# daisy9542/yolo-puncture

Measured on AMD Instinct MI355X. Metric: images/sec, higher is better.
Workload: dtype bf16

## Files before the change

### include/yolop.h

```cpp
#ifndef YOLOP_H
#define YOLOP_H

#include <stddef.h>
#include <stdint.h>

#ifdef __cplusplus
extern "C" {
#endif

#define YP_OK 0
#define YP_ERR_ARG -1
#define YP_ERR_STATE -2
#define YP_ERR_HIP -3
#define YP_ERR_WEIGHT -4

#define YP_BF16 0
#define YP_F32 1

#define YP_TASK_DETECT 0
#define YP_TASK_SEGMENT 1

#define YP_NM 32
#define YP_MAX_MASKS 480
#define YP_ID_MASKS_FRAMES_BUDGET (1ull << 30)
// ... 143 lines not shown
int yp_debug_op_cfg(const yp_engine* e, int i, int* cfg);
int yp_debug_last_store_form(void);
int yp_debug_max_workgroups(int n);
int yp_debug_conv_families(int* base, int* num_cfgs, int cap);
int yp_debug_ablation(int v);
int yp_debug_head_clocks(uint64_t* out8);
int yp_debug_attention(const void* qkv_dev, void* o_dev, int dtype, int B, int N, int nh, int kd, int hd, int q_stride, int q_coff, int o_stride,
                       int o_coff, int wgs, int* kernel_out, void* stream);
int yp_debug_attention_form(const void* qkv_dev, void* o_dev, int dtype, int B, int N, int nh, int kd, int hd, int q_stride, int q_coff, int o_stride,
                            int o_coff, int wgs, int form, int* kernel_out, void* stream);
int yp_debug_attention_f32(const void* qkv_dev, void* o_dev, int B, int N, int nh, int kd, int hd, int q_stride, int q_coff, int o_stride, int o_coff,
                           int wgs, int f32_stream, int* kernel_out, void* stream);
int yp_debug_conv_s2(const void* x_dev, const void* w_dev, const float* bias_dev, const void* res_dev, void* y_dev, int out_f32, int B, int H,
                     int W, int Cin, int Cout, int silu, int cfg, int lds_weights, int64_t* lds_out, char* kernel_out, int kernel_cap,
                     void* stream);
int yp_debug_topk_anchors(const uint32_t* const mk_dev[3], int B, const int hw[3][2], int k, int32_t* sel_out_dev, uint32_t* thr_out_dev, void* stream);
int yp_debug_head_branch_clocks(uint64_t* out8);
int yp_debug_head_winners(yp_engine* e, int32_t* sel_host, float* box_host, float* coeff_host);
int yp_debug_contour_clocks(uint64_t* out12);
int yp_debug_pwsp_clocks(uint64_t* out32);

int yp_tuning_source(const yp_engine* e);

int yp_debug_host_selftest(yp_engine* e);
int yp_debug_graph_info(const yp_engine* e, int64_t* out6);
int yp_debug_head_positions(yp_engine* e, int64_t* out6);
int yp_debug_marker(void* stream);

int yp_set_graph(yp_engine* e, int enable);

// ... 5 lines not shown
```

### yolo-puncture_amd/csrc/common.h

```cpp
#pragma once
#include <hip/hip_runtime.h>
#include <stdint.h>
#include <atomic>
#include <cstdlib>
#include <initializer_list>
#include <string>
#include <type_traits>
#include <vector>

namespace yp {

enum DType { DT_BF16 = 0, DT_F32 = 1 };
enum Act { ACT_NONE = 0, ACT_SILU = 1, ACT_RELU = 2 };

enum OpKind {
    OP_STEM = 0,
    OP_CONV = 1,
    OP_DWCONV = 2,
    OP_POOL5 = 3,
    OP_UPSAMPLE = 4,
    OP_ATTN = 5,
    OP_HEAD = 6,
    OP_CONVT = 7,
    OP_AMAX = 9,
// ... 297 lines not shown
template <class F> auto with_res_f32(const ConvParams& p, F f) {
    if (p.out_f32) return f(std::false_type{}, std::true_type{});
    if (p.res) return f(std::true_type{}, std::false_type{});
    return f(std::false_type{}, std::false_type{});
}
inline std::string res_f32_args(const ConvParams& p) { return with_res_f32(p, [](auto res, auto f32) { return bool_args({res, f32}); }); }
inline bool conv_store_side_ok(const ConvParams& p) {
    if ((p.Cout & 3) || (p.y_stride & 3) || (p.y_coff & 3) || (p.res && ((p.res_stride & 3) || (p.res_coff & 3)))) return false;
    if (p.res && p.out_f32) return false;
    return p.x_bytes < (1ull << 31) && p.w_bytes < (1ull << 31) && p.y_bytes < (1ull << 31);
}
extern const ConvFamily conv_dma_family, conv_halo_family, conv_halo_p_family, conv_dma_p_family, conv_dma_lc_family, conv_halo_s2_family,
    conv_tile1_family, conv_wreg_family, conv_pxd_family, conv_ks_family, conv_wres_family, conv_wrs_family;
constexpr int kNumConvFamilies = 12;
extern const ConvFamily* const kConvFamilies[kNumConvFamilies];
int conv_halo_s2_pw_cfg(const ConvParams& p);
size_t conv_halo_s2_lds_bytes(const ConvParams& p, int c);
int conv_halo_s2_lds_weights(int on);
hipError_t launch_dwconv(const DwParams& p, int dtype, hipStream_t st);
std::string dwconv_kernel_name(const DwParams& p, int dtype);
hipError_t launch_stem(const StemParams& p, int dtype, hipStream_t st);
std::string stem_kernel_name(const StemParams& p, int dtype);
hipError_t launch_pool5(const PoolParams& p, int dtype, hipStream_t st);
hipError_t launch_sppf_pool3(const PoolParams& p, int dtype, hipStream_t st);
bool sppf_pool3_fits(const PoolParams& p, int dtype);
bool dwconv_mfma_valid(const DwParams& p, int dtype);
hipError_t launch_dwconv_mfma(const DwParams& p, hipStream_t st);
const char* dwconv_mfma_kernel_name(const DwParams& p);
hipError_t launch_upsample(const UpParams& p, int dtype, hipStream_t st);
enum AttnForm { ATTN_FORM_AUTO = 0, ATTN_FORM_STREAM = 1, ATTN_FORM_STREAM_WIDE = 3 };
inline bool attn_form_valid(int form) { return form == ATTN_FORM_AUTO || form == ATTN_FORM_STREAM || form == ATTN_FORM_STREAM_WIDE; }
// ... 144 lines not shown
```

### yolo-puncture_amd/csrc/conv_halo_s2.hip

```cpp
#include "common.h"

namespace yp {

constexpr int kS2WregMaxVgprs = 144;

template <int FM, int FN, int WGM, int WGN, int NSH, bool HAS_RES, bool OUT_F32, bool PW2, int NCH>
__device__ __forceinline__ void conv_halo_s2_body(const ConvParams& p, const int tiles_h, const int tiles_w, const int ntiles, const int G) {
    constexpr int NW = WGM * WGN;
    constexpr int TH = WGM * FM, BN = WGN * FN * 16;
    constexpr int HR = 2 * TH + 1;
    constexpr int HP = HR * 33;
    constexpr int H_INSTR = (HP * 4 + 63) / 64;
    constexpr int LH = (H_INSTR + NW - 1) / NW;
    constexpr int HB = H_INSTR * 1024;
    constexpr int S = FM * FN;
    constexpr bool WREG = NCH > 0;
    static_assert(!WREG || (!PW2 && 9 * NCH * FN * 4 <= kS2WregMaxVgprs), "register-weights form");
    static_assert(NSH == 3, "wait selection below is written for a 3-slot ring");
    static_assert((NSH - 2) * LH + 2 * S < 64, "vmcnt immediate");

    extern __shared__ __attribute__((aligned(1024))) unsigned char smem[];
    unsigned char* const Hs = smem;
    unsigned char* const dump = smem + NSH * HB;
    unsigned char* const Wres = dump + 1024;

    const int tid = threadIdx.x, lane = tid & 63;
    const int wave = __builtin_amdgcn_readfirstlane(tid >> 6);
    const int wm = wave % WGM, wn = wave / WGM;
    const int fr = lane & 15, fc = lane >> 4;
    const int nchunk = WREG ? NCH : p.Cin >> 5;

    const int bid = xcd_remap(blockIdx.x, gridDim.x);
// ... 48 lines not shown
                for (int a = 0; a < FN; ++a) {
                    const int rw = t * BN + wn * (FN * 16) + a * 16 + fr;
                    wr[c][t][a] = *(const bf16x8*)(Hs + swz64((unsigned)(rw * 64 + fc * 16)));
                }
            __builtin_amdgcn_s_waitcnt(0xc07f);
            __builtin_amdgcn_s_barrier();
        }
#pragma unroll
        for (int c = 0; c < NCH; ++c)
#pragma unroll
            for (int t = 0; t < 9; ++t)
#pragma unroll
                for (int a = 0; a < FN; ++a) asm volatile("" : "+v"(wr[c][t][a]));
    }

    unsigned char* const W2s = Wres + (size_t)9 * nchunk * BN * 64;
    float bias2[FN][4];
    if (PW2) {
        static_assert(!PW2 || BN == 64, "the fused trailing 1x1 is written for a 64-wide intermediate and output");
        const __amdgpu_buffer_rsrc_t w2rs = __builtin_amdgcn_make_buffer_rsrc((void*)p.w2, 0, (int)p.w2_bytes, 0x00020000);
        for (int ii = wave; ii < BN * 8 / 64; ii += NW) {
            const int s = ii * 64 + lane;
            const int row = s >> 3, pc = s & 7;
            const int c8 = pc ^ ((row >> 1) & 7);
            const unsigned voff = (unsigned)((row * p.Kpad2 + c8 * 8) * 2);
            __builtin_amdgcn_raw_ptr_buffer_load_lds(w2rs, (lds_void*)(W2s + ii * 1024), 16, voff, 0, 0, 0);
        }
#pragma unroll
        for (int a = 0; a < FN; ++a) {
            const int co = wn * (FN * 16) + a * 16 + fc * 4;
#pragma unroll
            for (int r = 0; r < 4; ++r) bias2[a][r] = (co + r < p.C2) ? p.bias2[co + r] : 0.f;
        }
    }

    unsigned hconst[LH];
    auto set_tile = [&](int tile) {
        int t = tile;
        const int tw = t % tiles_w; t /= tiles_w;
// ... 108 lines not shown

        if (PW2) {
            unsigned char* tb = Hs + ((rd_slot == 0) ? NSH - 1 : rd_slot - 1) * HB;
            __builtin_amdgcn_s_barrier();
#pragma unroll
            for (int r = 0; r < FM; ++r) {
                const int px = (wm * FM + r) * 16 + fr;
#pragma unroll
                for (int a = 0; a < FN; ++a) {
                    const int co = wn * (FN * 16) + a * 16 + fc * 4;
                    __attribute__((aligned(8))) __bf16 o[4];
                    float sv[4] = {acc[a][r][0], acc[a][r][1], acc[a][r][2], acc[a][r][3]};
                    if (p.act == ACT_SILU) silu4_packed(sv);
#pragma unroll
                    for (int i = 0; i < 4; ++i) o[i] = (__bf16)sv[i];
                    asm volatile("ds_write_b64 %0, %1" ::"v"((unsigned)(size_t)(__attribute__((address_space(3))) unsigned char*)(tb + px * 128 + (((co >> 3) ^ ((px >> 1) & 7)) * 16) + (co & 7) * 2)),
                                 "v"(*(const unsigned long long*)o) : "memory");
                }
            }
            asm volatile("s_waitcnt lgkmcnt(0)" ::: "memory");
            __builtin_amdgcn_s_barrier();
#pragma unroll
            for (int a = 0; a < FN; ++a)
#pragma unroll
                for (int r = 0; r < FM; ++r) acc[a][r] = f32x4{bias2[a][0], bias2[a][1], bias2[a][2], bias2[a][3]};
#pragma unroll
            for (int ss = 0; ss < 2; ++ss) {
                bf16x8 w2f[FN], t2f[FM];
#pragma unroll
                for (int a = 0; a < FN; ++a) {
                    const int rw = wn * (FN * 16) + a * 16 + fr;
                    w2f[a] = *(const bf16x8*)(W2s + rw * 128 + (((ss * 4 + fc) ^ ((rw >> 1) & 7)) * 16));
                }
#pragma unroll
                for (int r = 0; r < FM; ++r) {
                    const int px = (wm * FM + r) * 16 + fr;
                    t2f[r] = *(const bf16x8*)(tb + px * 128 + (((ss * 4 + fc) ^ ((px >> 1) & 7)) * 16));
                }
#pragma unroll
                for (int a = 0; a < FN; ++a)
#pragma unroll
                    for (int r = 0; r < FM; ++r) acc[a][r] = __builtin_amdgcn_mfma_f32_16x16x32_bf16(w2f[a], t2f[r], acc[a][r], 0, 0, 0);
            }
        }
        {
            int t = tile;
            const int tw = t % tiles_w; t /= tiles_w;
            const int th = t % tiles_h;
            const int b = t / tiles_h;
            const int wo = tw * 16 + fr;
            uint2 rres[FM][FN];
            if (HAS_RES) {
// ... 41 lines not shown
    wait_vmcnt<0>();
}

template <int FM, int FN, int WGM, int WGN, int NSH, bool HAS_RES, bool OUT_F32, bool PW2>
__global__ __launch_bounds__(WGM * WGN * 64) void conv_halo_s2_kernel(const ConvParams p, const int tiles_h, const int tiles_w,
                                                                    const int ntiles, const int G) {
    conv_halo_s2_body<FM, FN, WGM, WGN, NSH, HAS_RES, OUT_F32, PW2, 0>(p, tiles_h, tiles_w, ntiles, G);
}
template <int FM, int FN, int WGM, int WGN, int NSH, bool HAS_RES, bool OUT_F32, bool PW2, int NCH>
__global__ __launch_bounds__(WGM * WGN * 64) void conv_halo_s2_kernel(const ConvParams p, const int tiles_h, const int tiles_w,
                                                                    const int ntiles, const int G) {
    static_assert(NCH > 0, "the ninth argument is a register-weights form's chunk count");
    conv_halo_s2_body<FM, FN, WGM, WGN, NSH, HAS_RES, OUT_F32, PW2, NCH>(p, tiles_h, tiles_w, ntiles, G);
}

enum { S2_PW2 = 1, S2_WREG = 2 };
template <int FM, int FN, int WGM, int WGN, int FORM = 0> struct S2 : Cfg<FM, FN, WGM, WGN, 3> {
    static constexpr int TH = WGM * FM, BN = WGN * FN * 16;
    static constexpr bool pw2 = FORM & S2_PW2, wreg = FORM & S2_WREG;
    static constexpr size_t lds(int Cin, bool with_pw2 = false) {
        const size_t ring = (size_t)3 * (((2 * TH + 1) * 33 * 4 + 63) / 64) * 1024 + 1024;
        if (wreg) return std::max(ring, (size_t)9 * BN * 64);
        return ring + (size_t)9 * (Cin / 32) * BN * 64 + (with_pw2 ? (size_t)BN * 128 : 0);
    }
};
using S2Forms = CfgList<
    S2<2, 2, 4, 2, S2_PW2>,
    S2<1, 2, 4, 2, S2_PW2>,
    S2<2, 2, 4, 1>,
    S2<1, 2, 4, 1>,
    S2<2, 4, 4, 2>,
    S2<1, 2, 4, 2, S2_WREG>,
    S2<2, 2, 4, 2, S2_WREG>,
    S2<2, 2, 2, 4, S2_WREG>>;
constexpr int kNumS2 = 5;

static std::atomic<int>& s2_lds_weights_ref() {
    static std::atomic<int> v{env_on("YOLOP_S2_LDS_WEIGHTS") ? 1 : 0};
    return v;
}
int conv_halo_s2_lds_weights(int on) { return on < 0 ? s2_lds_weights_ref().load() : s2_lds_weights_ref().exchange(on ? 1 : 0); }

static int halo_s2_form(const ConvParams& p, int c) {
    if (c < 0 || c >= kNumS2) return -1;
    if (c > 1 || p.C2 > 0 || s2_lds_weights_ref().load()) return c;
    if ((p.Cin % 32) != 0 || 9 * (p.Cin / 32) * 2 * 4 > kS2WregMaxVgprs) return c;
    if (c == 0) return 6;
    return p.Cout > 96 ? 7 : 5;
}
static std::string conv_halo_s2_symbol(const ConvParams& p, int c) {
    return with_cfg<S2Forms>(halo_s2_form(p, c), [&](auto k) {
        if (k.wreg) return cfg_symbol("conv_halo_s2_kernel", k, res_f32_args(p) + bool_args({false}) + "," + std::to_string(p.Cin / 32));
        return cfg_symbol("conv_halo_s2_kernel", k, p.C2 > 0 ? bool_args({false, false, true}) : res_f32_args(p) + bool_args({false}));
    });
}

static bool conv_halo_s2_cfg_valid(const ConvParams& p, int c) {
    if (p.ks != 3 || p.stride != 2 || p.pad != 1 || p.up != 1 || (p.Cin % 32) != 0 || (p.Kpad != 9 * p.Cin)) return false;
    if ((p.H & 1) || (p.W & 1) || p.Ho * 2 != p.H || p.Wo * 2 != p.W) return false;
    if (!conv_store_side_ok(p)) return false;
    return with_cfg<S2Forms>(halo_s2_form(p, c), [&](auto k) {
        using K = decltype(k);
        const int cpad = (p.Cout + 31) / 32 * 32;
        if (K::BN > cpad) return false;
        if (K::lds(p.Cin) > 160 * 1024) return false;
        const long covered = (long)((p.Ho + K::TH - 1) / K::TH * K::TH) * ((p.Wo + 15) / 16 * 16);
// ... 1 lines not shown
    });
}

template <bool HAS_RES, bool OUT_F32, bool PW2, int... WCH, int FM, int FN, int WGM, int WGN, int FORM>
static hipError_t launch_halo_s2_var(S2<FM, FN, WGM, WGN, FORM> k, const ConvParams& p, hipStream_t st) {
    static_assert(sizeof...(WCH) == 0 || (FN == 2 && 9 * 2 * FN * 4 <= kS2WregMaxVgprs && 9 * 3 * FN * 4 > kS2WregMaxVgprs), "the chunk counts instantiated are those halo_s2_form admits");
    constexpr int TH = k.TH, BN = k.BN;
    const size_t sh = k.lds(p.Cin, PW2);
    const int B = p.M / (p.Ho * p.Wo);
    const int tiles_h = (p.Ho + TH - 1) / TH, tiles_w = (p.Wo + 15) / 16, ntiles = (p.Cout + BN - 1) / BN;
    const int num_tiles = B * tiles_h * tiles_w;
    const int per_cu = sizeof...(WCH) > 0 ? 1 : (int)std::max<size_t>(1, std::min<size_t>(2, (160 * 1024) / sh));
    int G = (256 * per_cu) / ntiles;
    if (G < 1) G = 1;
    if (G > num_tiles) G = num_tiles;
    auto kern = conv_halo_s2_kernel<FM, FN, WGM, WGN, 3, HAS_RES, OUT_F32, PW2, WCH...>;
    static size_t granted = 0;
    if (hipError_t e = allow_dynamic_lds((const void*)kern, sh, granted)) return e;
    hipLaunchKernelGGL(kern, dim3(G * ntiles), dim3(WGM * WGN * 64), sh, st, p, tiles_h, tiles_w, ntiles, G);
    return hipGetLastError();
}

int conv_halo_s2_pw_cfg(const ConvParams& p) {
    if (p.w2 == nullptr && p.C2 == 0) return -1;
    if (p.Cout != 64 || p.C2 != 64 || p.Kpad2 != 64 || p.res || p.out_f32) return -1;
    for (int c : {0, 1}) {
        ConvParams q = p;
        q.Cout = p.C2;
        if (!conv_halo_s2_cfg_valid(q, c)) continue;
        if (with_cfg<S2Forms>(c, [&](auto k) { return k.lds(p.Cin, true); }) > 160 * 1024) continue;
        return c;
    }
    return -1;
}

size_t conv_halo_s2_lds_bytes(const ConvParams& p, int c) {
    return with_cfg<S2Forms>(halo_s2_form(p, c), [&](auto k) { return k.lds(p.Cin); });
}

static hipError_t launch_conv_halo_s2(const ConvParams& p, int c, hipStream_t st) {
    return with_cfg<S2Forms>(halo_s2_form(p, c), [&](auto k) {
        using K = decltype(k);
        if constexpr (K::wreg) {
            return with_res_f32(p, [&](auto res, auto f32) {
                if (p.Cin == 32) return launch_halo_s2_var<res, f32, false, 1>(k, p, st);
                if (p.Cin == 64) return launch_halo_s2_var<res, f32, false, 2>(k, p, st);
                return hipErrorInvalidValue;
            });
        } else {
            if (p.C2 > 0) {
                if constexpr (K::pw2) return launch_halo_s2_var<false, false, true>(k, p, st);
                else return hipErrorInvalidValue;
            }
            return with_res_f32(p, [&](auto res, auto f32) { return launch_halo_s2_var<res, f32, false>(k, p, st); });
        }
    });
}

// ... 6 lines not shown
```

### yolo-puncture_amd/csrc/engine.hip

```cpp
#include "../../include/yolop.h"
#include "common.h"
#include <algorithm>
#include <array>
#include <chrono>

#include <cmath>
#include <cstdarg>
#include <cstdio>
#include <cstring>
#include <cstdlib>
#include <dlfcn.h>
#include <fcntl.h>
#include <fstream>
#include <map>
#include <sstream>
#include <memory>

using namespace yp;

static thread_local char g_err[512] = "";
static int fail(int code, const char* fmt, ...) {
    va_list ap;
    va_start(ap, fmt);
    vsnprintf(g_err, sizeof(g_err), fmt, ap);
// ... 22 lines not shown
    size_t arena_bytes = 0;
    int proto_t = -1;
    void* mask_ws = nullptr;
    void* head_ws = nullptr;
    size_t head_ws_bytes = 0;
    size_t mask_ws_bytes = 0;
    bool use_graph = false;
    bool graph_auto = false;
    std::map<std::array<int, 3>, bool> auto_replay;
    bool fuse = true;
    int attn_form = ATTN_FORM_AUTO;
    int attn_f32_stream = ATTN_F32_GENERIC;
    bool tail = false;
    bool narrow_store = false;
    bool sparse_head = true;
    void* sp_ws = nullptr; size_t sp_ws_bytes = 0;
    bool tune = true;
    int tune_source = 0;
    hipStream_t own_stream = nullptr;
    hipEvent_t ev_in = nullptr;
    hipGraphExec_t gexec = nullptr;
    hipGraph_t gsrc = nullptr;
    bool use_lanes = true;
    int n_captures = 0;
    int g_nodes = 0, g_edges = 0, g_edges_expected = 0;
    hipStream_t last_stream = nullptr; bool have_last = false;
    struct LaneStep { int op = -1; std::vector<int> waits; bool fork = false; bool record = false; };
    std::vector<LaneStep> lane_steps;
    std::vector<int> lanes_used;
    int n_lanes = 1;
// ... 772 lines not shown

static int tail_absorbed(const yp_engine& e, const Op& o, int m[3]) {
    if (o.fuse_tail < 0) return 0;
    m[0] = e.ops[o.fuse_tail].fuse_dw; m[1] = o.fuse_tail; m[2] = o.tail_amax;
    return o.tail_amax >= 0 ? 3 : 2;
}
static std::string tail_admit(const yp_engine& e, const Op& o, int& cfg) {
    return e.tail && e.ops[o.fuse_tail].form == FORM_DWPW ? dwpw_admit(e, o, cfg) : "";
}
static void tail_views(const yp_engine& e, const Op& o, View& in, View& extra) {
    in = e.ops[e.ops[o.fuse_tail].fuse_dw].in;
    if (o.tail_amax >= 0) extra = e.ops[o.tail_amax].out;
}

static int s2pw_absorbed(const yp_engine&, const Op& o, int m[3]) { return link1(o.fuse_pre, m); }
static std::string s2pw_admit(const yp_engine& e, const Op& o, int& cfg) {
    const ConvParams q = conv_params(e, o);
    const int c = conv_halo_s2_pw_cfg(q);
    if (c < 0) return "";
    cfg = conv_halo_s2_family.base + c;
    return conv_halo_s2_family.symbol(q, c);
}
static void s2pw_views(const yp_engine& e, const Op& o, View& in, View&) { in = e.ops[o.fuse_pre].in; }
static hipError_t s2pw_launch(const yp_engine& e, const Op& o, const RunArgs&, hipStream_t st) {
    return conv_halo_s2_family.launch(conv_params(e, o), o.cfg - conv_halo_s2_family.base, st);
}

static int front_absorbed(const yp_engine&, const Op& o, int m[3]) {
    m[0] = o.stem_op; m[1] = o.fuse_pre;
    return o.stem_op >= 0 && o.fuse_pre >= 0 ? 2 : 0;
}
static std::string front_admit(const yp_engine& e, const Op& o, int&) {
    return e.weights[e.ops[o.stem_op].widx].d_w2 && frontend_valid(front_params(e, o, nullptr)) ? "frontend_kernel" : "";
// ... 959 lines not shown
    std::unique_ptr<yp_engine> e(new yp_engine());
    e->desc = *desc; e->device = device; e->dtype = desc->dtype;
    e->fuse = !env_on("YOLOP_NO_FUSE");
    e->tail = env_on("YOLOP_TAIL");
    if (const char* v = std::getenv("YOLOP_ATTN_FORM")) {
        if (!strcmp(v, "stream")) e->attn_form = ATTN_FORM_STREAM;
        else if (!strcmp(v, "stream_wide")) e->attn_form = ATTN_FORM_STREAM_WIDE;
        else if (*v && strcmp(v, "auto")) return fail(YP_ERR_ARG, "YOLOP_ATTN_FORM=%s (auto | stream | stream_wide)", v);
    }
    if (const char* v = std::getenv("YOLOP_ATTN_F32")) {
        if (!strcmp(v, "stream")) e->attn_f32_stream = ATTN_F32_STREAM;
        else if (!strcmp(v, "stream_wide")) e->attn_f32_stream = ATTN_F32_STREAM_WIDE;
        else if (*v) return fail(YP_ERR_ARG, "YOLOP_ATTN_F32=%s (stream | stream_wide, or unset)", v);
    }
    e->sparse_head = !env_on("YOLOP_DENSE_HEAD");
    e->narrow_store = env_on("YOLOP_NARROW_STORE");
    int rc = build_graph(*e);
    if (rc != YP_OK) return rc;
    for (const Op& o : e->ops)
        for (const View* v : {&o.in, &o.out, &o.res})
            if (v->t >= 0 && o.kind != OP_STEM && ((v->C & 7) || (v->coff & 7)) && !e->tensors[v->t].f32)
                return fail(YP_ERR_ARG, "op %s: channel slice (%d,%d) is not a multiple of 8", o.name.c_str(), v->coff, v->C);
    *out = e.release();
    return YP_OK;
}

int yp_destroy(yp_engine* e) {
    if (!e) return YP_OK;
    if (e->finalized || e->arena) { (void)hipSetDevice(e->device); (void)hipDeviceSynchronize(); }
    for (auto& w : e->weights) { if (w.d_w) (void)hipFree(w.d_w); if (w.d_w2) (void)hipFree(w.d_w2); if (w.d_b) (void)hipFree(w.d_b); }
// ... 600 lines not shown
    const int before = conv_halo_s2_lds_weights(lds_weights ? 1 : 0);
    const bool ok = f.valid(p, cfg - f.base);
    hipError_t err = hipSuccess;
    if (lds_out) *lds_out = (int64_t)conv_halo_s2_lds_bytes(p, cfg - f.base);
    if (ok && kernel_out && kernel_cap > 0) std::snprintf(kernel_out, (size_t)kernel_cap, "%s", f.symbol(p, cfg - f.base).c_str());
    if (ok && !host_only) {
        hipStream_t st = (hipStream_t)stream;
        err = f.launch(p, cfg - f.base, st);
        if (err == hipSuccess) err = hipStreamSynchronize(st);
    }
    conv_halo_s2_lds_weights(before);
    if (!ok)
        return fail(YP_ERR_ARG, "yp_debug_conv_s2: configuration %d does not admit B %d, H %d, W %d, Cin %d, Cout %d%s%s%s", cfg, B, H, W, Cin, Cout,
                    res_dev ? ", residual" : "", out_f32 ? ", fp32 output" : "", lds_weights ? ", weights in LDS" : "");
    if (err != hipSuccess) return fail(YP_ERR_HIP, "yp_debug_conv_s2: %s", hipGetErrorString(err));
    return YP_OK;
}

int yp_tuning_source(const yp_engine* e) {
    if (!e) return YP_ERR_ARG;
    return e->tune_source;
}

int yp_debug_graph_info(const yp_engine* e, int64_t* out6) {
    if (!e || !out6) return fail(YP_ERR_ARG, "yp_debug_graph_info: null argument");
    out6[0] = e->n_captures; out6[1] = e->g_nodes; out6[2] = e->g_edges; out6[3] = e->g_edges_expected;
    out6[4] = (int64_t)e->lanes_used.size() + 1; out6[5] = e->gexec ? 1 : 0;
    return YP_OK;
}

// ... 501 lines not shown
```

### yolo-puncture_amd/engine.py

```python
from __future__ import annotations

import ctypes as C
import os
from typing import Dict, List, Optional, Tuple

import numpy as np
import torch

from .weights import fold_state

_LIB: Optional[C.CDLL] = None
_HERE = os.path.dirname(os.path.abspath(__file__))
LIB_PATH = os.environ.get("YOLOP_LIB") or os.path.join(_HERE, "libyolop.so")

YP_BF16, YP_F32 = 0, 1
TASK_DETECT, TASK_SEGMENT = 0, 1
OP_KINDS = {0: "stem", 1: "conv", 2: "dwconv", 3: "pool5", 4: "upsample", 5: "attn", 6: "head", 7: "convT", 8: "pool3", 9: "amax"}
FORMS = ("plain", "dwpw", "dwpw_tail", "s2pw", "frontend", "c2f", "scdown", "pwsp", "cls_out")


class ModelDesc(C.Structure):
    _fields_ = [("variant", C.c_int), ("nc", C.c_int), ("task", C.c_int), ("dtype", C.c_int), ("max_det", C.c_int), ("family", C.c_int)]


# ... 31 lines not shown
    lib.yp_mask_contours_large_workspace.restype = C.c_size_t
    lib.yp_mask_contours_large.argtypes = [vp, C.c_int, C.c_int, C.c_int, C.c_int, C.c_int, vp, vp, vp, C.c_int, vp, C.c_int, C.c_int, C.c_int, vp,
                                           C.c_size_t, vp]
    lib.yp_mask_contours_large.restype = C.c_int
    lib.yp_plan.argtypes = [vp, C.c_int, C.c_int, C.c_int]
    lib.yp_max_batch.argtypes = [vp, C.c_int, C.c_int]
    lib.yp_max_batch.restype = C.c_int
    lib.yp_debug_topk_anchors.argtypes = [C.POINTER(vp), C.c_int, C.POINTER(C.c_int), C.c_int, vp, vp, vp]
    lib.yp_debug_topk_anchors.restype = C.c_int
    lib.yp_debug_attention.argtypes = [vp, vp] + [C.c_int] * 11 + [ip, vp]
    lib.yp_debug_attention.restype = C.c_int
    lib.yp_debug_attention_form.argtypes = [vp, vp] + [C.c_int] * 12 + [ip, vp]
    lib.yp_debug_attention_form.restype = C.c_int
    lib.yp_debug_conv_s2.argtypes = [vp, vp, vp, vp, vp] + [C.c_int] * 9 + [C.POINTER(C.c_int64), C.c_char_p, C.c_int, vp]
    lib.yp_debug_conv_s2.restype = C.c_int
    lib.yp_set_attention_form.argtypes = [vp, C.c_int]
    lib.yp_set_attention_form.restype = C.c_int
    lib.yp_debug_attention_f32.argtypes = [vp, vp] + [C.c_int] * 11 + [ip, vp]
    lib.yp_debug_attention_f32.restype = C.c_int
    lib.yp_set_attention_f32_stream.argtypes = [vp, C.c_int]
    lib.yp_set_attention_f32_stream.restype = C.c_int
    lib.yp_op_info.argtypes = [vp, C.c_int, C.c_char_p, C.c_int, ip, C.POINTER(C.c_double), C.POINTER(C.c_double)]
    lib.yp_op_output.argtypes = [vp, C.c_int, ip, ip, ip]
    lib.yp_op_kernel.argtypes = [vp, C.c_int, C.c_char_p, C.c_int]
    lib.yp_op_fusion.argtypes = [vp, C.c_int, ip, ip]
    lib.yp_op_fusion.restype = C.c_int
    lib.yp_debug_op_form.argtypes = [vp, C.c_int, ip, ip, C.c_int]
    lib.yp_debug_op_form.restype = C.c_int
    lib.yp_run_op.argtypes = [vp, C.c_int, vp, vp, vp, vp, vp]
    lib.yp_tensor_write.argtypes = [vp, C.c_int, C.c_int, C.c_int, vp]
# ... 50 lines not shown
    for fn in ("yp_comm_unique_id", "yp_comm_create", "yp_allgather", "yp_comm_destroy"):
        getattr(lib, fn).restype = C.c_int
    for fn in ("yp_create", "yp_destroy", "yp_weight_count", "yp_weight_info", "yp_set_weight", "yp_finalize",
               "yp_forward", "yp_proto", "yp_masks", "yp_plan", "yp_op_info", "yp_op_output", "yp_op_input", "yp_tensor_count",
               "yp_tensor_info", "yp_tensor_read", "yp_profile", "yp_set_graph", "yp_run_op", "yp_tensor_write",
               "yp_op_kernel", "yp_set_autotune", "yp_debug_force_conv_cfg", "yp_debug_ablation"):
        getattr(lib, fn).restype = C.c_int
    if path is None:
        _LIB = lib
    return lib


EXPORTS = ["yp_last_error", "yp_create", "yp_destroy", "yp_weight_count", "yp_weight_info", "yp_set_weight",
           "yp_finalize", "yp_forward", "yp_proto", "yp_masks", "yp_id_mask_resized", "yp_plan", "yp_op_info", "yp_op_output", "yp_op_input", "yp_op_fusion",
           "yp_tensor_count", "yp_tensor_info", "yp_tensor_read", "yp_profile", "yp_set_graph", "yp_run_op",
           "yp_tensor_write", "yp_op_kernel", "yp_set_autotune", "yp_tuning_export", "yp_tuning_import", "yp_set_nms", "yp_set_nms_options", "yp_debug_force_conv_cfg", "yp_debug_op_cfg", "yp_debug_op_form", "yp_debug_last_store_form", "yp_debug_max_workgroups", "yp_debug_conv_families", "yp_debug_ablation", "yp_debug_head_clocks", "yp_debug_head_branch_clocks", "yp_debug_head_winners", "yp_debug_contour_clocks", "yp_debug_pwsp_clocks", "yp_debug_host_selftest", "yp_debug_graph_info", "yp_tuning_source", "yp_debug_head_positions", "yp_debug_marker", "yp_max_batch", "yp_debug_topk_anchors", "yp_debug_attention", "yp_debug_attention_form", "yp_debug_attention_f32", "yp_debug_conv_s2", "yp_set_attention_form", "yp_set_attention_f32_stream", "yp_letterbox", "yp_letterbox_batch", "yp_masks_frames", "yp_masks_frames_input", "yp_id_masks_frames", "yp_id_masks_frames_workspace", "yp_mask_contours",
           "yp_mask_contours_scaled", "yp_mask_contours_large_workspace", "yp_mask_contours_large", "yp_comm_unique_id", "yp_comm_create", "yp_allgather", "yp_comm_destroy",
           "yp_u2net_create", "yp_u2net_destroy", "yp_u2net_weight_count", "yp_u2net_weight_info", "yp_u2net_set_weight", "yp_u2net_finalize",
           "yp_u2net_forward", "yp_u2net_forward_crops", "yp_u2net_set_graph", "yp_u2net_tensor_count", "yp_u2net_tensor_info", "yp_u2net_tensor_read",
           "yp_u2net_op_count", "yp_u2net_op_info",
           "yp_cls_create", "yp_cls_destroy", "yp_cls_weight_count", "yp_cls_weight_info", "yp_cls_set_weight", "yp_cls_finalize",
           "yp_cls_forward", "yp_cls_set_graph", "yp_cls_tensor_count", "yp_cls_tensor_info", "yp_cls_tensor_read"]


MAX_ANCHORS = 294912
MAX_MASKS = 480
ID_MASKS_FRAMES_BUDGET = 1 << 30
ATTENTION_FORMS = {"auto": 0, "stream": 1, "stream_wide": 3}


ATTENTION_F32 = {"generic": 0, "stream": 1}
# ... 88 lines not shown
                              C.c_void_p(res.data_ptr()) if res is not None else None, C.c_void_p(y.data_ptr()), int(bool(out_f32)), B, H, W, Cin, Cout,
                              int(bool(silu)), int(cfg), int(bool(lds_weights)), None, None, 0, C.c_void_p(_stream_ptr(x.device)))
    if rc < 0:
        raise YolopError(lib.yp_last_error().decode())
    return y


def conv_s2_admits(cfg: int, B: int, H: int, W: int, Cin: int, Cout: int, res: bool = False, out_f32: bool = False,
                   lds_weights: bool = False) -> Tuple[bool, int, str]:
    lib = load_library()
    lds = C.c_int64(0)
    name = C.create_string_buffer(160)
    rc = lib.yp_debug_conv_s2(None, None, None, C.c_void_p(1) if res else None, None, int(bool(out_f32)), int(B), int(H), int(W), int(Cin), int(Cout),
                              1, int(cfg), int(bool(lds_weights)), C.byref(lds), name, 160, None)
    return rc >= 0, int(lds.value), name.value.decode()


def conv_families() -> List[Tuple[int, int]]:
    lib = load_library()
    n = lib.yp_debug_conv_families(None, None, 0)
    base, num = (C.c_int * n)(), (C.c_int * n)()
    lib.yp_debug_conv_families(base, num, n)
    return list(zip(base, num))


def _stream_ptr(device: torch.device) -> int:
    return int(torch.cuda.current_stream(device).cuda_stream)


def letterbox_device(src: torch.Tensor, geo: dict, out: Optional[torch.Tensor] = None, pad_value: int = 114) -> torch.Tensor:
# ... 462 lines not shown
```

Measured before the change: 23610.

## Fuse trailing 128-wide 1x1 conv into register-weights stride-2 halo conv

Extends the stride-2 3x3 halo conv's fused trailing pointwise path from 64 to 128 intermediate/output channels (Cin 64). It adds a register-weights plus pw2 kernel variant that stages the tile intermediate through a halo slot and uses a swizzle sized for 128-wide rows. The goal is to drop the separate 1x1 conv launch and its intermediate global round-trip for these layers. It is gated on large tile counts and can be disabled by an env var; it costs extra LDS and register pressure. Debug entry points and Python bindings are added for testing.

New measurement: 23820 (median of 6 runs). Within noise of the previous version (+0.9%).

```diff
diff --git a/include/yolop.h b/include/yolop.h
--- a/include/yolop.h
+++ b/include/yolop.h
@@ -181,6 +181,11 @@
 int yp_debug_conv_s2(const void* x_dev, const void* w_dev, const float* bias_dev, const void* res_dev, void* y_dev, int out_f32, int B, int H,
                      int W, int Cin, int Cout, int silu, int cfg, int lds_weights, int64_t* lds_out, char* kernel_out, int kernel_cap,
                      void* stream);
+int yp_debug_conv_s2_pw(const void* x_dev, const void* w_dev, const float* bias_dev, const void* w2_dev, const float* bias2_dev, void* y_dev,
+                        int64_t y_bytes, int y_stride, int y_coff, int B, int H, int W, int Cin, int Cout, int C2, int silu, int silu2, int cfg,
+                        int64_t* lds_out, char* kernel_out, int kernel_cap, void* stream);
+int yp_debug_conv_pw(const void* x_dev, const void* w_dev, const float* bias_dev, void* y_dev, int64_t y_bytes, int y_stride, int y_coff, int B,
+                     int H, int W, int Cin, int Cout, int silu, int cfg, char* kernel_out, int kernel_cap, void* stream);
 int yp_debug_topk_anchors(const uint32_t* const mk_dev[3], int B, const int hw[3][2], int k, int32_t* sel_out_dev, uint32_t* thr_out_dev, void* stream);
 int yp_debug_head_branch_clocks(uint64_t* out8);
 int yp_debug_head_winners(yp_engine* e, int32_t* sel_host, float* box_host, float* coeff_host);
diff --git a/yolo-puncture_amd/csrc/common.h b/yolo-puncture_amd/csrc/common.h
--- a/yolo-puncture_amd/csrc/common.h
+++ b/yolo-puncture_amd/csrc/common.h
@@ -335,7 +335,7 @@
     conv_tile1_family, conv_wreg_family, conv_pxd_family, conv_ks_family, conv_wres_family, conv_wrs_family;
 constexpr int kNumConvFamilies = 12;
 extern const ConvFamily* const kConvFamilies[kNumConvFamilies];
-int conv_halo_s2_pw_cfg(const ConvParams& p);
+int conv_halo_s2_pw_cfg(const ConvParams& p, bool wide_ok = true);
 size_t conv_halo_s2_lds_bytes(const ConvParams& p, int c);
 int conv_halo_s2_lds_weights(int on);
 hipError_t launch_dwconv(const DwParams& p, int dtype, hipStream_t st);
diff --git a/yolo-puncture_amd/csrc/conv_halo_s2.hip b/yolo-puncture_amd/csrc/conv_halo_s2.hip
--- a/yolo-puncture_amd/csrc/conv_halo_s2.hip
+++ b/yolo-puncture_amd/csrc/conv_halo_s2.hip
@@ -15,7 +15,11 @@
     constexpr int HB = H_INSTR * 1024;
     constexpr int S = FM * FN;
     constexpr bool WREG = NCH > 0;
-    static_assert(!WREG || (!PW2 && 9 * NCH * FN * 4 <= kS2WregMaxVgprs), "register-weights form");
+    static_assert(!WREG || 9 * NCH * FN * 4 <= kS2WregMaxVgprs, "register-weights form");
+    static_assert(!PW2 || BN == 64 || BN == 128, "the fused trailing 1x1 is written for a 64- or 128-wide intermediate and output, one channel block");
+    static_assert(!PW2 || TH * 16 * BN * 2 <= HB, "the tile's intermediate goes through one halo slot");
+    constexpr int RB2 = BN * 2, CPR2 = RB2 / 16;
+    auto pw2_swz = [](int row) { return BN == 64 ? (row >> 1) & 7 : row & 15; };
     static_assert(NSH == 3, "wait selection below is written for a 3-slot ring");
     static_assert((NSH - 2) * LH + 2 * S < 64, "vmcnt immediate");
 
@@ -94,15 +98,15 @@
                 for (int a = 0; a < FN; ++a) asm volatile("" : "+v"(wr[c][t][a]));
     }
 
-    unsigned char* const W2s = Wres + (size_t)9 * nchunk * BN * 64;
+    constexpr size_t kStage = (size_t)NSH * HB + 1024 > (size_t)9 * BN * 64 ? (size_t)NSH * HB + 1024 : (size_t)9 * BN * 64;
+    unsigned char* const W2s = WREG ? smem + kStage : Wres + (size_t)9 * nchunk * BN * 64;
     float bias2[FN][4];
     if (PW2) {
-        static_assert(!PW2 || BN == 64, "the fused trailing 1x1 is written for a 64-wide intermediate and output");
         const __amdgpu_buffer_rsrc_t w2rs = __builtin_amdgcn_make_buffer_rsrc((void*)p.w2, 0, (int)p.w2_bytes, 0x00020000);
-        for (int ii = wave; ii < BN * 8 / 64; ii += NW) {
+        for (int ii = wave; ii < BN * CPR2 / 64; ii += NW) {
             const int s = ii * 64 + lane;
-            const int row = s >> 3, pc = s & 7;
-            const int c8 = pc ^ ((row >> 1) & 7);
+            const int row = s / CPR2, pc = s % CPR2;
+            const int c8 = pc ^ pw2_swz(row);
             const unsigned voff = (unsigned)((row * p.Kpad2 + c8 * 8) * 2);
             __builtin_amdgcn_raw_ptr_buffer_load_lds(w2rs, (lds_void*)(W2s + ii * 1024), 16, voff, 0, 0, 0);
         }
@@ -241,7 +245,7 @@
                     if (p.act == ACT_SILU) silu4_packed(sv);
 #pragma unroll
                     for (int i = 0; i < 4; ++i) o[i] = (__bf16)sv[i];
-                    asm volatile("ds_write_b64 %0, %1" ::"v"((unsigned)(size_t)(__attribute__((address_space(3))) unsigned char*)(tb + px * 128 + (((co >> 3) ^ ((px >> 1) & 7)) * 16) + (co & 7) * 2)),
+                    asm volatile("ds_write_b64 %0, %1" ::"v"((unsigned)(size_t)(__attribute__((address_space(3))) unsigned char*)(tb + px * RB2 + (((co >> 3) ^ pw2_swz(px)) * 16) + (co & 7) * 2)),
                                  "v"(*(const unsigned long long*)o) : "memory");
                 }
             }
@@ -252,17 +256,17 @@
 #pragma unroll
                 for (int r = 0; r < FM; ++r) acc[a][r] = f32x4{bias2[a][0], bias2[a][1], bias2[a][2], bias2[a][3]};
 #pragma unroll
-            for (int ss = 0; ss < 2; ++ss) {
+            for (int ss = 0; ss < BN / 32; ++ss) {
                 bf16x8 w2f[FN], t2f[FM];
 #pragma unroll
                 for (int a = 0; a < FN; ++a) {
                     const int rw = wn * (FN * 16) + a * 16 + fr;
-                    w2f[a] = *(const bf16x8*)(W2s + rw * 128 + (((ss * 4 + fc) ^ ((rw >> 1) & 7)) * 16));
+                    w2f[a] = *(const bf16x8*)(W2s + rw * RB2 + (((ss * 4 + fc) ^ pw2_swz(rw)) * 16));
                 }
 #pragma unroll
                 for (int r = 0; r < FM; ++r) {
                     const int px = (wm * FM + r) * 16 + fr;
-                    t2f[r] = *(const bf16x8*)(tb + px * 128 + (((ss * 4 + fc) ^ ((px >> 1) & 7)) * 16));
+                    t2f[r] = *(const bf16x8*)(tb + px * RB2 + (((ss * 4 + fc) ^ pw2_swz(px)) * 16));
                 }
 #pragma unroll
                 for (int a = 0; a < FN; ++a)
@@ -334,14 +338,21 @@
     conv_halo_s2_body<FM, FN, WGM, WGN, NSH, HAS_RES, OUT_F32, PW2, NCH>(p, tiles_h, tiles_w, ntiles, G);
 }
 
+template <int FM, int FN, int WGM, int WGN, int NSH, int NCH>
+__global__ __launch_bounds__(WGM * WGN * 64) void conv_halo_s2_pw_wide_kernel(const ConvParams p, const int tiles_h, const int tiles_w,
+                                                                            const int ntiles, const int G) {
+    static_assert(NCH > 0, "a register-weights form's chunk count");
+    conv_halo_s2_body<FM, FN, WGM, WGN, NSH, false, false, true, NCH>(p, tiles_h, tiles_w, ntiles, G);
+}
+
 enum { S2_PW2 = 1, S2_WREG = 2 };
 template <int FM, int FN, int WGM, int WGN, int FORM = 0> struct S2 : Cfg<FM, FN, WGM, WGN, 3> {
     static constexpr int TH = WGM * FM, BN = WGN * FN * 16;
     static constexpr bool pw2 = FORM & S2_PW2, wreg = FORM & S2_WREG;
     static constexpr size_t lds(int Cin, bool with_pw2 = false) {
         const size_t ring = (size_t)3 * (((2 * TH + 1) * 33 * 4 + 63) / 64) * 1024 + 1024;
-        if (wreg) return std::max(ring, (size_t)9 * BN * 64);
-        return ring + (size_t)9 * (Cin / 32) * BN * 64 + (with_pw2 ? (size_t)BN * 128 : 0);
+        if (wreg) return std::max(ring, (size_t)9 * BN * 64) + (pw2 ? (size_t)BN * BN * 2 : 0);
+        return ring + (size_t)9 * (Cin / 32) * BN * 64 + (with_pw2 ? (size_t)BN * BN * 2 : 0);
     }
 };
 using S2Forms = CfgList<
@@ -352,7 +363,8 @@
     S2<2, 4, 4, 2>,
     S2<1, 2, 4, 2, S2_WREG>,
     S2<2, 2, 4, 2, S2_WREG>,
-    S2<2, 2, 2, 4, S2_WREG>>;
+    S2<2, 2, 2, 4, S2_WREG>,
+    S2<2, 2, 2, 4, S2_WREG | S2_PW2>>;
 constexpr int kNumS2 = 5;
 
 static std::atomic<int>& s2_lds_weights_ref() {
@@ -363,13 +375,15 @@
 
 static int halo_s2_form(const ConvParams& p, int c) {
     if (c < 0 || c >= kNumS2) return -1;
-    if (c > 1 || p.C2 > 0 || s2_lds_weights_ref().load()) return c;
+    if (p.C2 > 0) return (c == 1 && p.Cin == 64 && p.Cout > 96) ? 8 : c;
+    if (c > 1 || s2_lds_weights_ref().load()) return c;
     if ((p.Cin % 32) != 0 || 9 * (p.Cin / 32) * 2 * 4 > kS2WregMaxVgprs) return c;
     if (c == 0) return 6;
     return p.Cout > 96 ? 7 : 5;
 }
 static std::string conv_halo_s2_symbol(const ConvParams& p, int c) {
     return with_cfg<S2Forms>(halo_s2_form(p, c), [&](auto k) {
+        if (k.wreg && k.pw2) return cfg_symbol("conv_halo_s2_pw_wide_kernel", k, "," + std::to_string(p.Cin / 32));
         if (k.wreg) return cfg_symbol("conv_halo_s2_kernel", k, res_f32_args(p) + bool_args({false}) + "," + std::to_string(p.Cin / 32));
         return cfg_symbol("conv_halo_s2_kernel", k, p.C2 > 0 ? bool_args({false, false, true}) : res_f32_args(p) + bool_args({false}));
     });
@@ -401,34 +415,41 @@
     int G = (256 * per_cu) / ntiles;
     if (G < 1) G = 1;
     if (G > num_tiles) G = num_tiles;
-    auto kern = conv_halo_s2_kernel<FM, FN, WGM, WGN, 3, HAS_RES, OUT_F32, PW2, WCH...>;
+    const void* kern;
+    if constexpr (PW2 && sizeof...(WCH) > 0) kern = (const void*)conv_halo_s2_pw_wide_kernel<FM, FN, WGM, WGN, 3, WCH...>;
+    else kern = (const void*)conv_halo_s2_kernel<FM, FN, WGM, WGN, 3, HAS_RES, OUT_F32, PW2, WCH...>;
     static size_t granted = 0;
-    if (hipError_t e = allow_dynamic_lds((const void*)kern, sh, granted)) return e;
-    hipLaunchKernelGGL(kern, dim3(G * ntiles), dim3(WGM * WGN * 64), sh, st, p, tiles_h, tiles_w, ntiles, G);
-    return hipGetLastError();
-}
-
-int conv_halo_s2_pw_cfg(const ConvParams& p) {
+    if (hipError_t e = allow_dynamic_lds(kern, sh, granted)) return e;
+    void* args[] = {(void*)&p, (void*)&tiles_h, (void*)&tiles_w, (void*)&ntiles, (void*)&G};
+    return hipLaunchKernel(kern, dim3(G * ntiles), dim3(WGM * WGN * 64), args, sh, st);
+}
+
+int conv_halo_s2_pw_cfg(const ConvParams& p, bool wide_ok) {
     if (p.w2 == nullptr && p.C2 == 0) return -1;
-    if (p.Cout != 64 || p.C2 != 64 || p.Kpad2 != 64 || p.res || p.out_f32) return -1;
+    if (p.res || p.out_f32) return -1;
+    const bool wide = p.Cin == 64 && p.Cout == 128 && p.C2 == 128 && p.Kpad2 == 128;
+    if (wide ? !wide_ok || s2_lds_weights_ref().load() != 0 : p.Cout != 64 || p.C2 != 64 || p.Kpad2 != 64) return -1;
     for (int c : {0, 1}) {
+        if (wide && c != 1) continue;
         ConvParams q = p;
         q.Cout = p.C2;
         if (!conv_halo_s2_cfg_valid(q, c)) continue;
-        if (with_cfg<S2Forms>(c, [&](auto k) { return k.lds(p.Cin, true); }) > 160 * 1024) continue;
+        if (with_cfg<S2Forms>(halo_s2_form(p, c), [&](auto k) { return k.lds(p.Cin, true); }) > 160 * 1024) continue;
         return c;
     }
     return -1;
 }
 
 size_t conv_halo_s2_lds_bytes(const ConvParams& p, int c) {
-    return with_cfg<S2Forms>(halo_s2_form(p, c), [&](auto k) { return k.lds(p.Cin); });
+    return with_cfg<S2Forms>(halo_s2_form(p, c), [&](auto k) { return k.lds(p.Cin, p.C2 > 0); });
 }
 
 static hipError_t launch_conv_halo_s2(const ConvParams& p, int c, hipStream_t st) {
     return with_cfg<S2Forms>(halo_s2_form(p, c), [&](auto k) {
         using K = decltype(k);
-        if constexpr (K::wreg) {
+        if constexpr (K::wreg && K::pw2) {
+            return p.C2 > 0 && p.Cin == 64 && !p.res && !p.out_f32 ? launch_halo_s2_var<false, false, true, 2>(k, p, st) : hipErrorInvalidValue;
+        } else if constexpr (K::wreg) {
             return with_res_f32(p, [&](auto res, auto f32) {
                 if (p.Cin == 32) return launch_halo_s2_var<res, f32, false, 1>(k, p, st);
                 if (p.Cin == 64) return launch_halo_s2_var<res, f32, false, 2>(k, p, st);
diff --git a/yolo-puncture_amd/csrc/engine.hip b/yolo-puncture_amd/csrc/engine.hip
--- a/yolo-puncture_amd/csrc/engine.hip
+++ b/yolo-puncture_amd/csrc/engine.hip
@@ -60,6 +60,7 @@
     bool tail = false;
     bool narrow_store = false;
     bool sparse_head = true;
+    bool s2pw_wide = true;
     void* sp_ws = nullptr; size_t sp_ws_bytes = 0;
     bool tune = true;
     int tune_source = 0;
@@ -862,9 +863,11 @@
 }
 
 static int s2pw_absorbed(const yp_engine&, const Op& o, int m[3]) { return link1(o.fuse_pre, m); }
+constexpr long kS2pwWideMinTiles = 1024;
 static std::string s2pw_admit(const yp_engine& e, const Op& o, int& cfg) {
     const ConvParams q = conv_params(e, o);
-    const int c = conv_halo_s2_pw_cfg(q);
+    const long tiles = (long)e.pB * ((q.Ho + 3) / 4) * ((q.Wo + 15) / 16);
+    const int c = conv_halo_s2_pw_cfg(q, e.s2pw_wide && o.stem_op < 0 && tiles >= kS2pwWideMinTiles);
     if (c < 0) return "";
     cfg = conv_halo_s2_family.base + c;
     return conv_halo_s2_family.symbol(q, c);
@@ -1854,6 +1857,7 @@
         else if (*v) return fail(YP_ERR_ARG, "YOLOP_ATTN_F32=%s (stream | stream_wide, or unset)", v);
     }
     e->sparse_head = !env_on("YOLOP_DENSE_HEAD");
+    e->s2pw_wide = !env_on("YOLOP_NO_S2PW_WIDE");
     e->narrow_store = env_on("YOLOP_NARROW_STORE");
     int rc = build_graph(*e);
     if (rc != YP_OK) return rc;
@@ -2484,6 +2488,76 @@
         return fail(YP_ERR_ARG, "yp_debug_conv_s2: configuration %d does not admit B %d, H %d, W %d, Cin %d, Cout %d%s%s%s", cfg, B, H, W, Cin, Cout,
                     res_dev ? ", residual" : "", out_f32 ? ", fp32 output" : "", lds_weights ? ", weights in LDS" : "");
     if (err != hipSuccess) return fail(YP_ERR_HIP, "yp_debug_conv_s2: %s", hipGetErrorString(err));
+    return YP_OK;
+}
+
+int yp_debug_conv_s2_pw(const void* x_dev, const void* w_dev, const float* bias_dev, const void* w2_dev, const float* bias2_dev, void* y_dev,
+                        int64_t y_bytes, int y_stride, int y_coff, int B, int H, int W, int Cin, int Cout, int C2, int silu, int silu2, int cfg,
+                        int64_t* lds_out, char* kernel_out, int kernel_cap, void* stream) {
+    if (lds_out) *lds_out = 0;
+    if (kernel_out && kernel_cap > 0) kernel_out[0] = 0;
+    const bool host_only = !x_dev && !w_dev && !bias_dev && !w2_dev && !bias2_dev && !y_dev;
+    if (!host_only && (!x_dev || !w_dev || !bias_dev || !w2_dev || !bias2_dev || !y_dev)) return fail(YP_ERR_ARG, "yp_debug_conv_s2_pw: null argument");
+    if (B < 1 || H < 2 || W < 2 || Cin < 1 || Cout < 1 || C2 < 1)
+        return fail(YP_ERR_ARG, "yp_debug_conv_s2_pw: non-positive size (B %d, H %d, W %d, Cin %d, Cout %d, C2 %d)", B, H, W, Cin, Cout, C2);
+    const ConvFamily& f = conv_halo_s2_family;
+    if (cfg != f.base && cfg != f.base + 1) return fail(YP_ERR_ARG, "yp_debug_conv_s2_pw: cfg = %d, the fused forms are ids %d and %d", cfg, f.base, f.base + 1);
+    ConvParams p{};
+    p.x = x_dev; p.x_stride = Cin; p.x_coff = 0; p.H = H; p.W = W; p.Cin = Cin;
+    p.w = w_dev; p.Kpad = 9 * Cin; p.bias = bias_dev;
+    p.Ho = H / 2; p.Wo = W / 2; p.Cout = Cout;
+    p.y = y_dev; p.y_stride = y_stride; p.y_coff = y_coff;
+    p.M = B * p.Ho * p.Wo;
+    p.ks = 3; p.stride = 2; p.pad = 1; p.up = 1;
+    p.act = silu ? ACT_SILU : ACT_NONE;
+    p.w2 = w2_dev; p.bias2 = bias2_dev; p.C2 = C2; p.act2 = silu2 ? ACT_SILU : ACT_NONE; p.Kpad2 = Cout; p.w2_bytes = (size_t)C2 * Cout * 2;
+    p.x_bytes = (size_t)B * H * W * Cin * 2; p.w_bytes = (size_t)Cout * 9 * Cin * 2; p.y_bytes = (size_t)std::max<int64_t>(y_bytes, 0);
+    p.cfg = -1;
+    if (y_stride < C2 || y_coff < 0 || ((int64_t)(p.M - 1) * y_stride + y_coff + C2) * 2 > y_bytes)
+        return fail(YP_ERR_ARG, "yp_debug_conv_s2_pw: the output slice (stride %d, offset %d, %d channels, %d pixels) does not lie in %lld bytes", y_stride,
+                    y_coff, C2, p.M, (long long)y_bytes);
+    const bool ok = conv_halo_s2_pw_cfg(p, !env_on("YOLOP_NO_S2PW_WIDE")) == cfg - f.base;
+    hipError_t err = hipSuccess;
+    if (lds_out) *lds_out = (int64_t)conv_halo_s2_lds_bytes(p, cfg - f.base);
+    if (ok && kernel_out && kernel_cap > 0) std::snprintf(kernel_out, (size_t)kernel_cap, "%s", f.symbol(p, cfg - f.base).c_str());
+    if (ok && !host_only) {
+        hipStream_t st = (hipStream_t)stream;
+        err = f.launch(p, cfg - f.base, st);
+        if (err == hipSuccess) err = hipStreamSynchronize(st);
+    }
+    if (!ok) return fail(YP_ERR_ARG, "yp_debug_conv_s2_pw: configuration %d does not admit B %d, H %d, W %d, Cin %d, Cout %d, C2 %d", cfg, B, H, W, Cin, Cout, C2);
+    if (err != hipSuccess) return fail(YP_ERR_HIP, "yp_debug_conv_s2_pw: %s", hipGetErrorString(err));
+    return YP_OK;
+}
+
+int yp_debug_conv_pw(const void* x_dev, const void* w_dev, const float* bias_dev, void* y_dev, int64_t y_bytes, int y_stride, int y_coff, int B,
+                     int H, int W, int Cin, int Cout, int silu, int cfg, char* kernel_out, int kernel_cap, void* stream) {
+    if (kernel_out && kernel_cap > 0) kernel_out[0] = 0;
+    if (!x_dev || !w_dev || !bias_dev || !y_dev) return fail(YP_ERR_ARG, "yp_debug_conv_pw: null argument");
+    if (B < 1 || H < 1 || W < 1 || Cin < 1 || Cout < 1) return fail(YP_ERR_ARG, "yp_debug_conv_pw: non-positive size (B %d, H %d, W %d, Cin %d, Cout %d)", B, H, W, Cin, Cout);
+    const ConvFamily* f = nullptr;
+    for (const ConvFamily* k : kConvFamilies)
+        if (cfg >= k->base && cfg < k->base + k->num_cfgs) f = k;
+    if (!f) return fail(YP_ERR_ARG, "yp_debug_conv_pw: cfg = %d is no id of a conv tile family", cfg);
+    ConvParams p{};
+    p.x = x_dev; p.x_stride = Cin; p.x_coff = 0; p.H = H; p.W = W; p.Cin = Cin;
+    p.w = w_dev; p.Kpad = Cin; p.bias = bias_dev;
+    p.Ho = H; p.Wo = W; p.Cout = Cout;
+    p.y = y_dev; p.y_stride = y_stride; p.y_coff = y_coff;
+    p.M = B * H * W;
+    p.ks = 1; p.stride = 1; p.pad = 0; p.up = 1; p.wide = 1;
+    p.act = silu ? ACT_SILU : ACT_NONE;
+    p.x_bytes = (size_t)p.M * Cin * 2; p.w_bytes = (size_t)Cout * Cin * 2; p.y_bytes = (size_t)std::max<int64_t>(y_bytes, 0);
+    p.cfg = cfg;
+    if (y_stride < Cout || y_coff < 0 || ((int64_t)(p.M - 1) * y_stride + y_coff + Cout) * 2 > y_bytes)
+        return fail(YP_ERR_ARG, "yp_debug_conv_pw: the output slice (stride %d, offset %d, %d channels, %d pixels) does not lie in %lld bytes", y_stride, y_coff,
+                    Cout, p.M, (long long)y_bytes);
+    if (!f->valid(p, cfg - f->base)) return fail(YP_ERR_ARG, "yp_debug_conv_pw: configuration %d does not admit B %d, H %d, W %d, Cin %d, Cout %d", cfg, B, H, W, Cin, Cout);
+    if (kernel_out && kernel_cap > 0) std::snprintf(kernel_out, (size_t)kernel_cap, "%s", f->symbol(p, cfg - f->base).c_str());
+    hipStream_t st = (hipStream_t)stream;
+    hipError_t err = f->launch(p, cfg - f->base, st);
+    if (err == hipSuccess) err = hipStreamSynchronize(st);
+    if (err != hipSuccess) return fail(YP_ERR_HIP, "yp_debug_conv_pw: %s", hipGetErrorString(err));
     return YP_OK;
 }
 
diff --git a/yolo-puncture_amd/engine.py b/yolo-puncture_amd/engine.py
--- a/yolo-puncture_amd/engine.py
+++ b/yolo-puncture_amd/engine.py
@@ -69,6 +69,10 @@
     lib.yp_debug_attention_form.restype = C.c_int
     lib.yp_debug_conv_s2.argtypes = [vp, vp, vp, vp, vp] + [C.c_int] * 9 + [C.POINTER(C.c_int64), C.c_char_p, C.c_int, vp]
     lib.yp_debug_conv_s2.restype = C.c_int
+    lib.yp_debug_conv_s2_pw.argtypes = [vp] * 6 + [C.c_int64] + [C.c_int] * 11 + [C.POINTER(C.c_int64), C.c_char_p, C.c_int, vp]
+    lib.yp_debug_conv_s2_pw.restype = C.c_int
+    lib.yp_debug_conv_pw.argtypes = [vp] * 4 + [C.c_int64] + [C.c_int] * 9 + [C.c_char_p, C.c_int, vp]
+    lib.yp_debug_conv_pw.restype = C.c_int
     lib.yp_set_attention_form.argtypes = [vp, C.c_int]
     lib.yp_set_attention_form.restype = C.c_int
     lib.yp_debug_attention_f32.argtypes = [vp, vp] + [C.c_int] * 11 + [ip, vp]
@@ -149,7 +153,7 @@
 EXPORTS = ["yp_last_error", "yp_create", "yp_destroy", "yp_weight_count", "yp_weight_info", "yp_set_weight",
            "yp_finalize", "yp_forward", "yp_proto", "yp_masks", "yp_id_mask_resized", "yp_plan", "yp_op_info", "yp_op_output", "yp_op_input", "yp_op_fusion",
            "yp_tensor_count", "yp_tensor_info", "yp_tensor_read", "yp_profile", "yp_set_graph", "yp_run_op",
-           "yp_tensor_write", "yp_op_kernel", "yp_set_autotune", "yp_tuning_export", "yp_tuning_import", "yp_set_nms", "yp_set_nms_options", "yp_debug_force_conv_cfg", "yp_debug_op_cfg", "yp_debug_op_form", "yp_debug_last_store_form", "yp_debug_max_workgroups", "yp_debug_conv_families", "yp_debug_ablation", "yp_debug_head_clocks", "yp_debug_head_branch_clocks", "yp_debug_head_winners", "yp_debug_contour_clocks", "yp_debug_pwsp_clocks", "yp_debug_host_selftest", "yp_debug_graph_info", "yp_tuning_source", "yp_debug_head_positions", "yp_debug_marker", "yp_max_batch", "yp_debug_topk_anchors", "yp_debug_attention", "yp_debug_attention_form", "yp_debug_attention_f32", "yp_debug_conv_s2", "yp_set_attention_form", "yp_set_attention_f32_stream", "yp_letterbox", "yp_letterbox_batch", "yp_masks_frames", "yp_masks_frames_input", "yp_id_masks_frames", "yp_id_masks_frames_workspace", "yp_mask_contours",
+           "yp_tensor_write", "yp_op_kernel", "yp_set_autotune", "yp_tuning_export", "yp_tuning_import", "yp_set_nms", "yp_set_nms_options", "yp_debug_force_conv_cfg", "yp_debug_op_cfg", "yp_debug_op_form", "yp_debug_last_store_form", "yp_debug_max_workgroups", "yp_debug_conv_families", "yp_debug_ablation", "yp_debug_head_clocks", "yp_debug_head_branch_clocks", "yp_debug_head_winners", "yp_debug_contour_clocks", "yp_debug_pwsp_clocks", "yp_debug_host_selftest", "yp_debug_graph_info", "yp_tuning_source", "yp_debug_head_positions", "yp_debug_marker", "yp_max_batch", "yp_debug_topk_anchors", "yp_debug_attention", "yp_debug_attention_form", "yp_debug_attention_f32", "yp_debug_conv_s2", "yp_debug_conv_s2_pw", "yp_debug_conv_pw", "yp_set_attention_form", "yp_set_attention_f32_stream", "yp_letterbox", "yp_letterbox_batch", "yp_masks_frames", "yp_masks_frames_input", "yp_id_masks_frames", "yp_id_masks_frames_workspace", "yp_mask_contours",
            "yp_mask_contours_scaled", "yp_mask_contours_large_workspace", "yp_mask_contours_large", "yp_comm_unique_id", "yp_comm_create", "yp_allgather", "yp_comm_destroy",
            "yp_u2net_create", "yp_u2net_destroy", "yp_u2net_weight_count", "yp_u2net_weight_info", "yp_u2net_set_weight", "yp_u2net_finalize",
            "yp_u2net_forward", "yp_u2net_forward_crops", "yp_u2net_set_graph", "yp_u2net_tensor_count", "yp_u2net_tensor_info", "yp_u2net_tensor_read",
@@ -268,6 +272,52 @@
     rc = lib.yp_debug_conv_s2(None, None, None, C.c_void_p(1) if res else None, None, int(bool(out_f32)), int(B), int(H), int(W), int(Cin), int(Cout),
                               1, int(cfg), int(bool(lds_weights)), C.byref(lds), name, 160, None)
     return rc >= 0, int(lds.value), name.value.decode()
+
+
+def conv_s2_pw(x: torch.Tensor, w: torch.Tensor, bias: torch.Tensor, w2: torch.Tensor, bias2: torch.Tensor, cfg: int, out: torch.Tensor,
+               guard_rows: int = 0, coff: int = 0, silu: bool = True, silu2: bool = True) -> None:
+    lib = load_library()
+    ts = (x, w, bias, w2, bias2, out)
+    if not all(t.is_cuda and t.is_contiguous() for t in ts) or any(t.dtype != torch.bfloat16 for t in (x, w, w2, out)) or \
+            bias.dtype != torch.float32 or bias2.dtype != torch.float32 or x.dim() != 4 or w.dim() != 4 or w2.dim() != 2 or out.dim() != 2:
+        raise ValueError("contiguous device tensors: bf16 x [B, H, W, Cin], w [Cout, 3, 3, Cin], w2 [C2, Cout], out [rows, stride]; float32 biases")
+    B, H, W, Cin = (int(v) for v in x.shape)
+    Cout, C2, stride = int(w.shape[0]), int(w2.shape[0]), int(out.shape[1])
+    if tuple(w.shape) != (Cout, 3, 3, Cin) or tuple(w2.shape) != (C2, Cout) or tuple(bias.shape) != (Cout,) or tuple(bias2.shape) != (C2,):
+        raise ValueError("w must be [Cout, 3, 3, Cin], w2 [C2, Cout], bias [Cout], bias2 [C2]")
+    rc = lib.yp_debug_conv_s2_pw(C.c_void_p(x.data_ptr()), C.c_void_p(w.data_ptr()), C.c_void_p(bias.data_ptr()), C.c_void_p(w2.data_ptr()),
+                                 C.c_void_p(bias2.data_ptr()), C.c_void_p(out.data_ptr()), int(out.numel()) * 2, stride,
+                                 int(guard_rows) * stride + int(coff), B, H, W, Cin, Cout, C2, int(bool(silu)), int(bool(silu2)), int(cfg),
+                                 None, None, 0, C.c_void_p(_stream_ptr(x.device)))
+    if rc < 0:
+        raise YolopError(lib.yp_last_error().decode())
+
+
+def conv_s2_pw_admits(cfg: int, B: int, H: int, W: int, Cin: int, Cout: int, C2: int) -> Tuple[bool, int, str]:
+    lib = load_library()
+    lds = C.c_int64(0)
+    name = C.create_string_buffer(160)
+    M = int(B) * (int(H) // 2) * (int(W) // 2)
+    rc = lib.yp_debug_conv_s2_pw(None, None, None, None, None, None, M * int(C2) * 2, int(C2), 0, int(B), int(H), int(W), int(Cin), int(Cout),
+                                 int(C2), 1, 1, int(cfg), C.byref(lds), name, 160, None)
+    return rc >= 0, int(lds.value), name.value.decode()
+
+
+def conv_pw(x: torch.Tensor, w: torch.Tensor, bias: torch.Tensor, cfg: int, out: torch.Tensor, guard_rows: int = 0, coff: int = 0,
+            silu: bool = True) -> str:
+    lib = load_library()
+    if not all(t.is_cuda and t.is_contiguous() for t in (x, w, bias, out)) or any(t.dtype != torch.bfloat16 for t in (x, w, out)) or \
+            bias.dtype != torch.float32 or x.dim() != 4 or out.dim() != 2 or tuple(w.shape) != (int(bias.shape[0]), int(x.shape[3])):
+        raise ValueError("contiguous device tensors: bf16 x [B, H, W, Cin], w [Cout, Cin], out [rows, stride]; float32 bias [Cout]")
+    B, H, W, Cin = (int(v) for v in x.shape)
+    stride = int(out.shape[1])
+    name = C.create_string_buffer(160)
+    rc = lib.yp_debug_conv_pw(C.c_void_p(x.data_ptr()), C.c_void_p(w.data_ptr()), C.c_void_p(bias.data_ptr()), C.c_void_p(out.data_ptr()),
+                              int(out.numel()) * 2, stride, int(guard_rows) * stride + int(coff), B, H, W, Cin, int(w.shape[0]), int(bool(silu)),
+                              int(cfg), name, 160, C.c_void_p(_stream_ptr(x.device)))
+    if rc < 0:
+        raise YolopError(lib.yp_last_error().decode())
+    return name.value.decode()
 
 
 def conv_families() -> List[Tuple[int, int]]:
```
